# fudan-zvg/S-NeRF

Measured on AMD Instinct MI355X. Metric: rays/sec (train step), higher is better.
Workload: dtype bf16; 1 GPU; S-NeRF path A (MipNerfModel) train step, nuScenes-like 1600x900 rays, 64 proposal + 128 fine evals/ray (192 spp), hidden 1024, rgb_layer 3, cone + contraction + IPE-96

## Files before the change

### snerf_amd/csrc/gemm.hip

```cpp
#include "common.h"
#include <cstdlib>
#include <type_traits>

#define ACT_NONE 0
#define ACT_RELU 1
#define ACT_MASK 2
typedef unsigned short u16x2 __attribute__((ext_vector_type(2)));
#define ACT_RELU_BITS 3
#define ACT_MASK_BITS 4

typedef unsigned u32x4 __attribute__((ext_vector_type(4)));
typedef unsigned u32x2 __attribute__((ext_vector_type(2)));

struct GemmNT {
  const void* A; long lda;
  const void* W; long ldw;
  const float* bias;
  void* Y; long ldy;
  const void* aux; long ldaux;
  float* colsum;
  int M, N, K, n_store, act, out_f32, vec_store;
  float* colsum_ws; int fast_epi;
  int det;
  int dbg;
  int stagger;
  int split;
  int aux_split;
};
__device__ __forceinline__ int split_a_tile(int v) { return 2 * (v / 3) + (v % 3 == 1 ? 1 : 0); }
#ifndef SNERF_PROBE
#define SNERF_PROBE 0
#endif
#define DBG(p, bit) (SNERF_PROBE && ((p).dbg & (bit)))

template <typename T> struct Frag;
template <> struct Frag<float> { typedef f32x4 type; };
template <> struct Frag<__bf16> { typedef bf16x8 type; };

__device__ __forceinline__ void mma32(f32x16& acc, const bf16x8& a, const bf16x8& b) {
  acc = __builtin_amdgcn_mfma_f32_32x32x16_bf16(a, b, acc, 0, 0, 0);
}
__device__ __forceinline__ void mma32(f32x16& acc, const f32x4& a, const f32x4& b) {
#pragma unroll
  for (int s = 0; s < 4; ++s) acc = __builtin_amdgcn_mfma_f32_32x32x2f32(a[s], b[s], acc, 0, 0, 0);
}

typedef _Float16 f16x8 __attribute__((ext_vector_type(8)));
template <bool F16> __device__ __forceinline__ void mma32t(f32x16& acc, const bf16x8& a, const bf16x8& b) {
  if constexpr (F16) acc = __builtin_amdgcn_mfma_f32_32x32x16_f16(__builtin_bit_cast(f16x8, a), __builtin_bit_cast(f16x8, b), acc, 0, 0, 0);
  else acc = __builtin_amdgcn_mfma_f32_32x32x16_bf16(a, b, acc, 0, 0, 0);
}
template <bool F16> __device__ __forceinline__ void mma32t(f32x16& acc, const f32x4& a, const f32x4& b) { mma32(acc, a, b); }
typedef int i32x8 __attribute__((ext_vector_type(8)));
__device__ __forceinline__ void mma8(f32x16& acc, const bf16x8& a0, const bf16x8& a1, const bf16x8& b0, const bf16x8& b1) {
  const i32x8 a = __builtin_bit_cast(i32x8, __builtin_shufflevector(a0, a1, 0, 1, 2, 3, 4, 5, 6, 7, 8, 9, 10, 11, 12, 13, 14, 15));
  const i32x8 b = __builtin_bit_cast(i32x8, __builtin_shufflevector(b0, b1, 0, 1, 2, 3, 4, 5, 6, 7, 8, 9, 10, 11, 12, 13, 14, 15));
  acc = __builtin_amdgcn_mfma_scale_f32_32x32x64_f8f6f4(a, b, acc, 0, 0, 0, 0x74747474, 0, 0x74747474);
}
template <bool F16> __device__ __forceinline__ __bf16 cvt16(float v) {
  if constexpr (F16) return __builtin_bit_cast(__bf16, (_Float16)v);
  else return (__bf16)v;
}
template <bool F16> __device__ __forceinline__ float up16(__bf16 h) {
  if constexpr (F16) return (float)__builtin_bit_cast(_Float16, h);
  else return (float)h;
}
template <bool F16> __device__ __forceinline__ float up16(float x) { return x; }
template <typename T, bool F16> __device__ __forceinline__ T down16(float v) {
  if constexpr (sizeof(T) == 4) return v;
  else return cvt16<F16>(v);
}

typedef __attribute__((address_space(3))) void* lds_ptr_t;
typedef const __attribute__((address_space(1))) void* gbl_ptr_t;

__device__ __forceinline__ void glds16(const void* g, char* lds_wave_base) {
  __builtin_amdgcn_global_load_lds((gbl_ptr_t)g, (lds_ptr_t)lds_wave_base, 16, 0, 0);
}

template <typename T, int BM, int BN, int WM, int WN, bool F16 = false>
__device__ __forceinline__ void nt_epilogue(const GemmNT& p, f32x16 (&acc)[BM / WM / 32][BN / WN / 32], char* smem,
                                            const int m0, const int n0, const int wave, const int lane) {
  typedef typename Frag<T>::type frag_t;
  constexpr int EPC = 16 / (int)sizeof(T);
  constexpr int WTM = BM / WM, WTN = BN / WN, TM = WTM / 32, TN = WTN / 32;
// ... 1150 lines not shown
  variant &= 15;
  hipStream_t s = (hipStream_t)stream;
  const bool p8 = dtype == SNERF_DT_BF16 && (variant & 8) && N % 256 == 0 && K >= 128 && fast && !(colsum != nullptr && act == ACT_RELU) &&
                  (lda * 2 * 256 < (1L << 31)) && (ldw * 2 * 256 < (1L << 31)) && !(split && (act == ACT_MASK || (colsum != nullptr && act == ACT_RELU_BITS))) &&
                  !aux_split &&
                  !(split == 2 && K < 256);
  if (act >= ACT_RELU_BITS && !(p8 && (long)((M + 255) / 256) * 8 * (N / 64) * 256 < (1L << 31)))
    return SNERF_ERR_ARG;
  if (f16) {
    if (p8) return launch_nt8p<true>(p, s);
    if (split == 2) return launch_nt<__bf16, 128, 128, 2, 2, true>(p, s);
    if ((variant & 12) && N % 256 == 0) return launch_nt8<true>(p, s);
    if ((variant & 1) && N % 256 == 0) return launch_nt<__bf16, 256, 256, 2, 4, true>(p, s);
    return launch_nt<__bf16, 128, 128, 2, 2, true>(p, s);
  }
  if (p8) return launch_nt8p(p, s);
  if (dtype == SNERF_DT_BF16 && (variant & 12) && N % 256 == 0) return launch_nt8(p, s);
  if (dtype == SNERF_DT_F32) return launch_nt<float, 128, 128, 2, 2>(p, s);
  if ((variant & 1) && N % 256 == 0) return launch_nt<__bf16, 256, 256, 2, 4>(p, s);
  return launch_nt<__bf16, 128, 128, 2, 2>(p, s);
}

struct GemmTN {
  const void* Z; long ldz;
  const void* X; long ldx;
  float* dW; long ldw;
  const void* zeros;
  int M, N, K, n_valid, k_valid, m_chunk;
  int tiles, slices;
  int split;
  float* part;
  long part_stride;
  int part_ld;
};

template <typename T, bool TR, int TN_STAGES, bool F16 = false>
__global__ __launch_bounds__(256) void gemm_tn_kernel(GemmTN p) {
  extern __shared__ __attribute__((aligned(16))) char smem[];
  constexpr int EPC = 16 / (int)sizeof(T);
  constexpr int ROWB = 128 * (int)sizeof(T);
  constexpr int MT = sizeof(T) == 4 ? 16 : 32;
  constexpr int TILEB = MT * ROWB;
  constexpr int RPI = 1024 / ROWB;
  constexpr int LI = MT / RPI / 4;
  const int tid = threadIdx.x, lane = tid & 63;
  const int wave = __builtin_amdgcn_readfirstlane(tid >> 6);
  const int wn = wave >> 1, wk = wave & 1;
  const int tiles_k = (p.K + 127) / 128;
  const int ntile = p.tiles;
  int slice, tile;
  {
    const int b = (int)blockIdx.x, xcd = b & 7, idx = b >> 3;
    const int full = p.slices >> 3;
    const int extra = p.slices & 7;
    const int mine = full + (xcd < extra ? 1 : 0);
    if (idx >= mine * ntile) return;
    slice = (idx / ntile) * 8 + xcd;
    tile = idx % ntile;
  }
  const int n0 = (tile / tiles_k) * 128, k0 = (tile % tiles_k) * 128;
  const int mbeg = slice * p.m_chunk;
  const int mend = min(p.M, mbeg + p.m_chunk);
  const T* __restrict__ Z = (const T*)p.Z;
  const T* __restrict__ X = (const T*)p.X;
  const int steps = (mend - mbeg + MT - 1) / MT;

// ... 86 lines not shown
        for (int t = 0; t < 2; ++t) {
          const int ca = (wn * 64 + t * 32 + (lane & 31)) * 2, cb = (wk * 64 + t * 32 + (lane & 31)) * 2;
#pragma unroll
          for (int e = 0; e < 8; ++e) {
            a[t].u[e] = *(const unsigned short*)(sZ + (rbase + e) * ROWB + ca);
            b[t].u[e] = *(const unsigned short*)(sX + (rbase + e) * ROWB + cb);
          }
        }
#pragma unroll
        for (int i = 0; i < 2; ++i)
#pragma unroll
          for (int j = 0; j < 2; ++j) mma32t<F16>(acc[i][j], a[i].v, b[j].v);
      }
    }
  }
#pragma unroll
  for (int i = 0; i < 2; ++i)
#pragma unroll
    for (int j = 0; j < 2; ++j) {
      int k = k0 + wk * 64 + j * 32 + (lane & 31);
      if (p.split == 1) k = ((k >> 7) << 6) | (k & 63);
#pragma unroll
      for (int r = 0; r < 16; ++r) {
        int n = n0 + wn * 64 + i * 32 + (r & 3) + 8 * (r >> 2) + 4 * (lane >> 5);
        if (p.split == 1) n = ((n >> 7) << 6) | (n & 63);
        if (n < p.n_valid && k < p.k_valid) {
          if (p.part != nullptr) p.part[(long)slice * p.part_stride + (long)n * p.part_ld + k] = acc[i][j][r];
          else atomicAdd(p.dW + (long)n * p.ldw + k, acc[i][j][r]);
        }
      }
    }
}

template <bool SPLIT, bool F16 = false>
__global__ __launch_bounds__(512) void gemm_tn8_kernel(GemmTN p) {
  extern __shared__ __attribute__((aligned(16))) char smem[];
  typedef __bf16 T;
  typedef __attribute__((address_space(3))) bf16x4* lds_b4;
  constexpr int HALF = 64 * 256;
  const int tid = threadIdx.x, lane = tid & 63;
  const int wave = __builtin_amdgcn_readfirstlane(tid >> 6);
  const int wr = wave >> 2, wc = wave & 3;
  const int tiles_k = (p.K + 255) >> 8, tiles_n = (p.N + 255) >> 8;
  const int ntile = tiles_k * tiles_n;
  const int id = xcd_remap((int)blockIdx.x, (int)gridDim.x);
  const int tile = id % ntile, chunk = id / ntile;
  const int n0 = (tile / tiles_k) << 8, k0 = (tile % tiles_k) << 8;
  const int mbeg = chunk * p.m_chunk;
  const int rows = min(p.M, mbeg + p.m_chunk) - mbeg;
  const int KT = (rows + 63) >> 6;
  const T* __restrict__ Z = (const T*)p.Z + (long)mbeg * p.ldz + n0;
  const bool xhi = !SPLIT && p.split == 2;
  const T* __restrict__ X = (const T*)p.X + (long)mbeg * p.ldx + (xhi ? 2 * k0 : k0);
  const int xcols = xhi ? ((p.K - 1) >> 6) * 128 + ((p.K - 1) & 63) + 1 - 2 * k0 : p.K - k0;
  const int zbytes = (rows - 1) * (int)p.ldz * 2 + (p.N - n0) * 2, xbytes = (rows - 1) * (int)p.ldx * 2 + xcols * 2;
  const int zstep = 64 * (int)p.ldz * 2, xstep = 64 * (int)p.ldx * 2;

  const int lrow = lane >> 4, lch = lane & 15;
  const int lc = (lch ^ (4 * lrow)) * 8;
  constexpr int xhalf = SPLIT ? 128 : 64;
  const int zcol = ((lc >> 6) * 128 + (lc & 63)) * 2;
  const int xcol = SPLIT ? (((lc >> 6) * 128) + ((lc >> 5) & 1) * 32 + (lc & 31)) * 2 : ((lc >> 5) * (xhi ? 128 : 64) + (lc & 31)) * 2;
  int zrel[2], xrel[2];
#pragma unroll
  for (int i = 0; i < 2; ++i) {
    const int r = (wave * 2 + i) * 4 + lrow;
    zrel[i] = r * (int)p.ldz * 2 + zcol;
    xrel[i] = r * (int)p.ldx * 2 + xcol;
  }
  int s_kt = 0;
  auto stage = [&](int db, int which) __attribute__((always_inline)) {
    char* dst = smem + (db * 4 + which) * HALF + wave * 2048;
    if (which < 2) {
      const int off = s_kt * zstep;
      const int left = zbytes - off;
      const __amdgpu_buffer_rsrc_t r = __builtin_amdgcn_make_buffer_rsrc((void*)((const char*)Z + off), 0, left > 0 ? left : 0, 0x00020000);
      __builtin_amdgcn_raw_ptr_buffer_load_lds(r, (lds_ptr_t)dst, 16, zrel[0] + which * 128, 0, 0, 0);
      __builtin_amdgcn_raw_ptr_buffer_load_lds(r, (lds_ptr_t)(dst + 1024), 16, zrel[1] + which * 128, 0, 0, 0);
    } else {
      const int off = s_kt * xstep;
      const int left = xbytes - off;
      const __amdgpu_buffer_rsrc_t r = __builtin_amdgcn_make_buffer_rsrc((void*)((const char*)X + off), 0, left > 0 ? left : 0, 0x00020000);
      __builtin_amdgcn_raw_ptr_buffer_load_lds(r, (lds_ptr_t)dst, 16, xrel[0] + (which - 2) * xhalf, 0, 0, 0);
      __builtin_amdgcn_raw_ptr_buffer_load_lds(r, (lds_ptr_t)(dst + 1024), 16, xrel[1] + (which - 2) * xhalf, 0, 0, 0);
    }
  };

  const int g4 = lane >> 4, pl = lane & 15, prow = pl >> 2;
  const int frow = (8 * (g4 >> 1) + prow) * 256;
  const int fsub = ((pl & 1) << 3);
  int zc[2], xc1;
#pragma unroll
  for (int i2 = 0; i2 < 2; ++i2) zc[i2] = ((((wr * 64 + i2 * 32 + 16 * (g4 & 1)) >> 3) + ((pl & 3) >> 1)) ^ (4 * prow)) << 4;
  xc1 = ((((wc * 32 + 16 * (g4 & 1)) >> 3) + ((pl & 3) >> 1)) ^ (4 * prow)) << 4;
  bf16x8 aF[2][4], bS[2][4];
  const unsigned lds0 = (unsigned)(size_t)smem;
  auto lds_frag = [&](unsigned addr) __attribute__((always_inline)) {
    bf16x4 lo, hi;
    asm volatile("ds_read_b64_tr_b16 %0, %2\n\tds_read_b64_tr_b16 %1, %2 offset:1024" : "=&v"(lo), "=&v"(hi) : "v"(addr));
    return __builtin_shufflevector(lo, hi, 0, 1, 2, 3, 4, 5, 6, 7);
  };
  const unsigned za[2] = {lds0 + frow + zc[0] + fsub, lds0 + frow + zc[1] + fsub};
  const unsigned xa = lds0 + frow + xc1 + fsub;
  auto lds_a = [&](int db, int h, int i2, int ks) __attribute__((always_inline)) {
    return lds_frag(za[i2] + (db * 4 + h) * HALF + ks * 4096);
  };
  auto lds_b = [&](int db, int g, int ks) __attribute__((always_inline)) {
    return lds_frag(xa + (db * 4 + 2 + g) * HALF + ks * 4096);
  };
  f32x16 acc[4][2];
#pragma unroll
  for (int i = 0; i < 4; ++i)
#pragma unroll
    for (int j = 0; j < 2; ++j)
#pragma unroll
      for (int r = 0; r < 16; ++r) acc[i][j][r] = 0.f;

  auto wait_load = [&]() __attribute__((always_inline)) {
    asm volatile("s_waitcnt vmcnt(10)" ::: "memory");
    __builtin_amdgcn_s_waitcnt(0xC07F);
    __builtin_amdgcn_sched_barrier(0);
  };
  auto end_phase = [&]() __attribute__((always_inline)) {
    __builtin_amdgcn_sched_barrier(0);
    __builtin_amdgcn_s_barrier();
    __builtin_amdgcn_sched_barrier(0);
  };

  stage(0, 2); stage(0, 0); stage(0, 3); stage(0, 1);
  ++s_kt;
  stage(1, 3); stage(1, 0); stage(1, 2); stage(1, 1);
  ++s_kt;
  asm volatile("s_waitcnt vmcnt(10)" ::: "memory");
  __builtin_amdgcn_s_barrier();
#pragma unroll
  for (int ks = 0; ks < 4; ++ks) {
    aF[0][ks] = lds_a(0, 0, 0, ks);
    aF[1][ks] = lds_a(0, 0, 1, ks);
    bS[0][ks] = lds_b(0, 0, ks);
  }
  __builtin_amdgcn_s_waitcnt(0xC07F);
  __builtin_amdgcn_sched_barrier(0);
  __builtin_amdgcn_s_barrier();

  auto ktile = [&](auto db_tag) __attribute__((always_inline)) {
    constexpr int db = decltype(db_tag)::value;
    constexpr int F = db, S = 1 - db;
    if (wr == 1) { stage(db, 2 + F); wait_load(); }
#pragma unroll
    for (int ks = 0; ks < 4; ++ks) {
      bS[S][ks] = lds_b(db, S, ks);
      mma32t<F16>(acc[0][F], aF[0][ks], bS[F][ks]);
      mma32t<F16>(acc[1][F], aF[1][ks], bS[F][ks]);
      __builtin_amdgcn_sched_barrier(0);
    }
    if (wr == 0) { stage(db, 2 + F); wait_load(); }
    end_phase();
    if (wr == 1) { stage(db, 0); wait_load(); }
#pragma unroll
    for (int ks = 0; ks < 4; ++ks)
#pragma unroll
      for (int i2 = 0; i2 < 2; ++i2) {
        mma32t<F16>(acc[i2][S], aF[i2][ks], bS[S][ks]);
        aF[i2][ks] = lds_a(db, 1, i2, ks);
        __builtin_amdgcn_sched_barrier(0);
      }
    if (wr == 0) { stage(db, 0); wait_load(); }
    end_phase();
    if (wr == 1) { stage(db, 2 + S); wait_load(); }
    constexpr bool skip3 = S == 1 && SPLIT, skip4 = F == 1 && SPLIT;
#pragma unroll
    for (int ks = 0; ks < 4; ++ks) {
      if constexpr (!skip3) {
        mma32t<F16>(acc[2][S], aF[0][ks], bS[S][ks]);
        mma32t<F16>(acc[3][S], aF[1][ks], bS[S][ks]);
      }
      bS[S][ks] = lds_b(db ^ 1, S, ks);
      __builtin_amdgcn_sched_barrier(0);
    }
    if (wr == 0) { stage(db, 2 + S); wait_load(); }
    end_phase();
    if (wr == 1) { stage(db, 1); ++s_kt; wait_load(); }
#pragma unroll
    for (int ks = 0; ks < 4; ++ks)
#pragma unroll
      for (int i2 = 0; i2 < 2; ++i2) {
        if constexpr (!skip4) mma32t<F16>(acc[2 + i2][F], aF[i2][ks], bS[F][ks]);
        aF[i2][ks] = lds_a(db ^ 1, 0, i2, ks);
        __builtin_amdgcn_sched_barrier(0);
      }
    if (wr == 0) { stage(db, 1); ++s_kt; wait_load(); }
    end_phase();
  };
  for (int t = 0; t < KT; t += 2) {
    ktile(std::integral_constant<int, 0>{});
    if (t + 1 < KT) ktile(std::integral_constant<int, 1>{});
  }
  asm volatile("s_waitcnt vmcnt(0)" ::: "memory");

#pragma unroll
  for (int i = 0; i < 4; ++i)
#pragma unroll
    for (int j = 0; j < 2; ++j) {
      int k = k0 + wc * 64 + j * 32 + (lane & 31);
      if constexpr (SPLIT) {
        if (i >= 2 && j == 1) continue;
        k = k0 + (wc >> 1) * 128 + j * 64 + (wc & 1) * 32 + (lane & 31);
        k = ((k >> 7) << 6) | (k & 63);
      }
#pragma unroll
      for (int r = 0; r < 16; ++r) {
        int n = n0 + wr * 128 + i * 32 + (r & 3) + 8 * (r >> 2) + 4 * (lane >> 5);
        if constexpr (SPLIT) n = ((n >> 7) << 6) | (n & 63);
        if (n < p.n_valid && k < p.k_valid) {
          if (p.part != nullptr) p.part[(long)chunk * p.part_stride + (long)n * p.part_ld + k] = acc[i][j][r];
          else atomicAdd(p.dW + (long)n * p.ldw + k, acc[i][j][r]);
        }
      }
    }
}

template <bool VEC>
__global__ __launch_bounds__(256) void tn_fold_kernel(const float* __restrict__ part, long part_stride, int part_ld, int slices, int n_valid,
                                                      int k_valid, float* __restrict__ dW, long ldw) {
  const int k = (blockIdx.x * 256 + threadIdx.x) * (VEC ? 4 : 1), n = blockIdx.y;
  if (k >= k_valid || n >= n_valid) return;
  const float* src = part + (long)n * part_ld + k;
  if constexpr (VEC) {
    f32x4 s = {0.f, 0.f, 0.f, 0.f};
#pragma unroll 8
    for (int c = 0; c < slices; ++c) s += *(const f32x4*)(src + (long)c * part_stride);
    f32x4* dst = (f32x4*)(dW + (long)n * ldw + k);
    *dst += s;
  } else {
    float s = 0.f;
    for (int c = 0; c < slices; ++c) s += src[(long)c * part_stride];
    dW[(long)n * ldw + k] += s;
  }
}

template <bool VEC>
__global__ __launch_bounds__(1024) void tn_fold_many_kernel(const float* __restrict__ part, long part_stride, int part_ld, int slices, int n_valid,
                                                            int k_valid, float* __restrict__ dW, long ldw) {
  constexpr int G = 16, W = VEC ? 4 : 1;
  __shared__ float sm[G][64][W];
  const int lane = threadIdx.x & 63, g = threadIdx.x >> 6;
  const int kq = k_valid / W;
  const long e = (long)blockIdx.x * 64 + lane;
  const bool live = e < (long)n_valid * kq;
  const int n = live ? (int)(e / kq) : 0, k = live ? (int)(e - (long)n * kq) * W : 0;
  const float* src = part + (long)n * part_ld + k;
  float s[W];
#pragma unroll
  for (int w = 0; w < W; ++w) s[w] = 0.f;
  if (live) {
#pragma unroll 4
    for (int c = g; c < slices; c += G) {
      if constexpr (VEC) { const f32x4 v = *(const f32x4*)(src + (long)c * part_stride); s[0] += v[0]; s[1] += v[1]; s[2] += v[2]; s[3] += v[3]; }
      else s[0] += src[(long)c * part_stride];
    }
  }
#pragma unroll
  for (int w = 0; w < W; ++w) sm[g][lane][w] = s[w];
  __syncthreads();
  if (g == 0 && live) {
    float* dst = dW + (long)n * ldw + k;
#pragma unroll
    for (int w = 0; w < W; ++w) {
      float t = sm[0][lane][w];
#pragma unroll
      for (int q = 1; q < G; ++q) t += sm[q][lane][w];
      dst[w] += t;
    }
  }
}

struct TnPlan {
  bool use8;
  int slices;
  int m_chunk;
  int part_ld;
  long part_stride;
};

static TnPlan tn_plan(int M, int N, int K, long ldz, long ldx, int dtype, int variant, bool fold = false) {
  static int n_cu = 0;
  if (n_cu == 0) {
    int dev = 0;
    hipDeviceProp_t prop;
    n_cu = 256;
    if (hipGetDevice(&dev) == hipSuccess && hipGetDeviceProperties(&prop, dev) == hipSuccess && prop.multiProcessorCount > 0)
      n_cu = prop.multiProcessorCount;
  }
  TnPlan pl{};
  if ((variant & 2) && dtype == SNERF_DT_BF16 && N % 256 == 0 && K >= 256 && M >= 4096 && ldz * 2 * 65 < (1L << 31) && ldx * 2 * 65 < (1L << 31)) {
    const int t8 = (N / 256) * ((K + 255) / 256);
    int ch = n_cu / t8;
    ch = ch < 1 ? 1 : ch;
    long mc = ((long)M + ch - 1) / ch;
    mc = ((mc + 127) / 128) * 128;
    const long lim = (1L << 30) / ((ldz > ldx ? ldz : ldx) * 2);
    if (mc > lim) mc = lim / 128 * 128;
    if (!(fold && M <= 131072 && mc < 512)) {
      pl.use8 = true; pl.m_chunk = (int)mc; pl.slices = (int)((M + mc - 1) / mc);
      pl.part_ld = ((K + 255) / 256) * 256; pl.part_stride = (long)N * pl.part_ld;
      return pl;
    }
  }
  const int tiles = ((N + 127) / 128) * ((K + 127) / 128);
  const int target = (variant & 64) ? 4096 : (variant & 32) ? 2048 : (variant & 16) ? 512 : 1024;
  int chunks = (target + tiles - 1) / tiles;
  int m_chunk = (M + chunks - 1) / chunks;
  m_chunk = ((m_chunk + 255) / 256) * 256;
  const int floor_rows = (fold && M <= 131072) ? 256 : 1024;
  if (m_chunk < floor_rows) m_chunk = floor_rows;
  pl.use8 = false; pl.m_chunk = m_chunk; pl.slices = (M + m_chunk - 1) / m_chunk;
  pl.part_ld = ((K + 127) / 128) * 128; pl.part_stride = (long)(((N + 127) / 128) * 128) * pl.part_ld;
  return pl;
}

static int wgrad_launch(const void* Z, long ldz, const void* X, long ldx, float* dW, long ldw, const void* zeros, int M, int N, int K,
                        int n_valid, int k_valid, int dtype, int variant, float* ws, long ws_floats, void* stream) {
  if (M <= 0) return SNERF_OK;
  const int split = dtype == SNERF_DT_BF16X3;
  if (split) {
    if (N % 128 != 0 || K % 128 != 0 || ws != nullptr) return SNERF_ERR_ARG;
    dtype = SNERF_DT_BF16;
  }
  const int xhi = (variant >> 14) & 1;
  if (xhi && (split || (dtype != SNERF_DT_BF16 && dtype != 2))) return SNERF_ERR_ARG;
  const bool f16 = dtype == 2;
  if (f16) dtype = SNERF_DT_BF16;
  const int epc = dtype == SNERF_DT_F32 ? 4 : 8;
  if (N < epc || K < epc || N % epc || K % epc || ldz % epc || ldx % epc || zeros == nullptr) return SNERF_ERR_ARG;
  const TnPlan pl = tn_plan(M, N, K, ldz, ldx, dtype, variant, ws != nullptr);
  if (ws != nullptr && ws_floats < pl.part_stride * pl.slices) return SNERF_ERR_ARG;
  GemmTN p{Z, ldz, X, ldx, dW, ldw, zeros, M, N, K, n_valid, k_valid, pl.m_chunk, 0, pl.slices, split ? 1 : (xhi ? 2 : 0), ws, pl.part_stride, pl.part_ld};
  if (pl.use8) {
    static bool attr_set = false;
    if (!attr_set) {
      hipFuncSetAttribute((const void*)gemm_tn8_kernel<false>, hipFuncAttributeMaxDynamicSharedMemorySize, 8 * 64 * 256);
      hipFuncSetAttribute((const void*)gemm_tn8_kernel<true>, hipFuncAttributeMaxDynamicSharedMemorySize, 8 * 64 * 256);
      attr_set = true;
    }
    const int t8 = (N / 256) * ((K + 255) / 256);
    if (f16) {
      static bool attr16 = false;
      if (!attr16) { hipFuncSetAttribute((const void*)gemm_tn8_kernel<false, true>, hipFuncAttributeMaxDynamicSharedMemorySize, 8 * 64 * 256); attr16 = true; }
      hipLaunchKernelGGL((gemm_tn8_kernel<false, true>), dim3(t8 * pl.slices), dim3(512), 8 * 64 * 256, (hipStream_t)stream, p);
    } else if (split) hipLaunchKernelGGL(gemm_tn8_kernel<true>, dim3(t8 * pl.slices), dim3(512), 8 * 64 * 256, (hipStream_t)stream, p);
    else hipLaunchKernelGGL(gemm_tn8_kernel<false>, dim3(t8 * pl.slices), dim3(512), 8 * 64 * 256, (hipStream_t)stream, p);
  } else {
    const int tiles = ((N + 127) / 128) * ((K + 127) / 128);
    p.tiles = tiles;
    const bool deep = (variant & 128) != 0;
    const int lds = (deep ? 4 : 2) * 2 * 8192;
    static bool tn_attr_set = false;
    if (!tn_attr_set) {
      hipFuncSetAttribute((const void*)gemm_tn_kernel<float, false, 4>, hipFuncAttributeMaxDynamicSharedMemorySize, 4 * 2 * 8192);
      hipFuncSetAttribute((const void*)gemm_tn_kernel<__bf16, true, 4>, hipFuncAttributeMaxDynamicSharedMemorySize, 4 * 2 * 8192);
      hipFuncSetAttribute((const void*)gemm_tn_kernel<__bf16, false, 4>, hipFuncAttributeMaxDynamicSharedMemorySize, 4 * 2 * 8192);
      tn_attr_set = true;
    }
    dim3 grid(8 * ((pl.slices + 7) / 8) * tiles);
    const bool tr = (variant & 1) && dtype == SNERF_DT_BF16 && (N % 128 == 0) && (K % 128 == 0);
    hipStream_t st = (hipStream_t)stream;
    if (f16) {
      static bool tn16_attr = false;
      if (!tn16_attr) {
        hipFuncSetAttribute((const void*)gemm_tn_kernel<__bf16, true, 4, true>, hipFuncAttributeMaxDynamicSharedMemorySize, 4 * 2 * 8192);
        hipFuncSetAttribute((const void*)gemm_tn_kernel<__bf16, false, 4, true>, hipFuncAttributeMaxDynamicSharedMemorySize, 4 * 2 * 8192);
        tn16_attr = true;
      }
      if (tr) { if (deep) hipLaunchKernelGGL((gemm_tn_kernel<__bf16, true, 4, true>), grid, dim3(256), lds, st, p);
                else hipLaunchKernelGGL((gemm_tn_kernel<__bf16, true, 2, true>), grid, dim3(256), lds, st, p); }
      else { if (deep) hipLaunchKernelGGL((gemm_tn_kernel<__bf16, false, 4, true>), grid, dim3(256), lds, st, p);
             else hipLaunchKernelGGL((gemm_tn_kernel<__bf16, false, 2, true>), grid, dim3(256), lds, st, p); }
    } else if (dtype == SNERF_DT_F32) {
      if (deep) hipLaunchKernelGGL((gemm_tn_kernel<float, false, 4>), grid, dim3(256), lds, st, p);
      else hipLaunchKernelGGL((gemm_tn_kernel<float, false, 2>), grid, dim3(256), lds, st, p);
    } else if (dtype == SNERF_DT_BF16 && tr) {
      if (deep) hipLaunchKernelGGL((gemm_tn_kernel<__bf16, true, 4>), grid, dim3(256), lds, st, p);
      else hipLaunchKernelGGL((gemm_tn_kernel<__bf16, true, 2>), grid, dim3(256), lds, st, p);
    } else if (dtype == SNERF_DT_BF16) {
      if (deep) hipLaunchKernelGGL((gemm_tn_kernel<__bf16, false, 4>), grid, dim3(256), lds, st, p);
      else hipLaunchKernelGGL((gemm_tn_kernel<__bf16, false, 2>), grid, dim3(256), lds, st, p);
    } else return SNERF_ERR_ARG;
  }
  if (ws != nullptr) {
    const bool vec = k_valid % 4 == 0 && pl.part_ld % 4 == 0 && pl.part_stride % 4 == 0 && ldw % 4 == 0 && ((size_t)dW & 15) == 0 && ((size_t)ws & 15) == 0;
    if (pl.slices > 32) {
      const long pieces = (long)n_valid * (vec ? k_valid / 4 : k_valid);
      const dim3 fg((unsigned)((pieces + 63) / 64));
      if (vec) hipLaunchKernelGGL(tn_fold_many_kernel<true>, fg, dim3(1024), 0, (hipStream_t)stream, ws, pl.part_stride, pl.part_ld, pl.slices, n_valid, k_valid, dW, ldw);
      else hipLaunchKernelGGL(tn_fold_many_kernel<false>, fg, dim3(1024), 0, (hipStream_t)stream, ws, pl.part_stride, pl.part_ld, pl.slices, n_valid, k_valid, dW, ldw);
    } else if (vec)
      hipLaunchKernelGGL(tn_fold_kernel<true>, dim3((k_valid / 4 + 255) / 256, n_valid), dim3(256), 0, (hipStream_t)stream, ws, pl.part_stride,
                         pl.part_ld, pl.slices, n_valid, k_valid, dW, ldw);
    else
      hipLaunchKernelGGL(tn_fold_kernel<false>, dim3((k_valid + 255) / 256, n_valid), dim3(256), 0, (hipStream_t)stream, ws, pl.part_stride,
                         pl.part_ld, pl.slices, n_valid, k_valid, dW, ldw);
  }
  return snerf_check_launch();
}

extern "C" int snerf_linear_wgrad(const void* Z, long ldz, const void* X, long ldx, float* dW, long ldw, const void* zeros,
                                  int M, int N, int K, int n_valid, int k_valid, int dtype, int variant, void* stream) {
  return wgrad_launch(Z, ldz, X, ldx, dW, ldw, zeros, M, N, K, n_valid, k_valid, dtype, variant, nullptr, 0, stream);
}

extern "C" long snerf_linear_wgrad_ws_floats(int M, int N, int K, long ldz, long ldx, int dtype, int variant) {
  if (M <= 0 || N <= 0 || K <= 0) return 0;
  if (dtype == 2) dtype = SNERF_DT_BF16;
  const TnPlan pl = tn_plan(M, N, K, ldz, ldx, dtype, variant, true);
  return pl.part_stride * pl.slices;
}

extern "C" int snerf_linear_wgrad_det(const void* Z, long ldz, const void* X, long ldx, float* dW, long ldw, const void* zeros, int M, int N,
                                      int K, int n_valid, int k_valid, int dtype, int variant, float* ws, long ws_floats, void* stream) {
  if (ws == nullptr) return SNERF_ERR_ARG;
  return wgrad_launch(Z, ldz, X, ldx, dW, ldw, zeros, M, N, K, n_valid, k_valid, dtype, variant, ws, ws_floats, stream);
}
```

Before: 162,800 rays/s.

## Schedule ragged-K edge tiles separately in bf16 weight-gradient GEMM

When K is not a multiple of 256 (remainder at most 128), the tn8 weight-gradient kernel now gives the partial last K tile its own blocks. These use a dedicated edge path that loads half-width X columns and skips MFMAs for dead wave columns. A planner picks separate M-chunk counts for full and edge tiles so the grid better fills the CUs, and the fold kernels sum a different slice count for the edge columns. The goal is to stop wasting half of each edge tile's MMA work and to balance load, at the cost of more planner complexity and a possibly larger workspace.

```diff
diff --git a/snerf_amd/csrc/gemm.hip b/snerf_amd/csrc/gemm.hip
--- a/snerf_amd/csrc/gemm.hip
+++ b/snerf_amd/csrc/gemm.hip
@@ -1,4 +1,5 @@
 #include "common.h"
+#include <climits>
 #include <cstdlib>
 #include <type_traits>
 
@@ -1267,6 +1268,7 @@
   float* part;
   long part_stride;
   int part_ld;
+  int edge_first, m_chunk_edge;
 };
 
 template <typename T, bool TR, int TN_STAGES, bool F16 = false>
@@ -1419,22 +1421,16 @@
     }
 }
 
-template <bool SPLIT, bool F16 = false>
-__global__ __launch_bounds__(512) void gemm_tn8_kernel(GemmTN p) {
-  extern __shared__ __attribute__((aligned(16))) char smem[];
+template <bool SPLIT, bool F16, bool EDGE>
+__device__ __forceinline__ void gemm_tn8_tile(const GemmTN& p, char* smem, const int n0, const int k0, const int chunk, const int m_chunk) {
   typedef __bf16 T;
   typedef __attribute__((address_space(3))) bf16x4* lds_b4;
   constexpr int HALF = 64 * 256;
   const int tid = threadIdx.x, lane = tid & 63;
   const int wave = __builtin_amdgcn_readfirstlane(tid >> 6);
   const int wr = wave >> 2, wc = wave & 3;
-  const int tiles_k = (p.K + 255) >> 8, tiles_n = (p.N + 255) >> 8;
-  const int ntile = tiles_k * tiles_n;
-  const int id = xcd_remap((int)blockIdx.x, (int)gridDim.x);
-  const int tile = id % ntile, chunk = id / ntile;
-  const int n0 = (tile / tiles_k) << 8, k0 = (tile % tiles_k) << 8;
-  const int mbeg = chunk * p.m_chunk;
-  const int rows = min(p.M, mbeg + p.m_chunk) - mbeg;
+  const int mbeg = chunk * m_chunk;
+  const int rows = min(p.M, mbeg + m_chunk) - mbeg;
   const int KT = (rows + 63) >> 6;
   const T* __restrict__ Z = (const T*)p.Z + (long)mbeg * p.ldz + n0;
   const bool xhi = !SPLIT && p.split == 2;
@@ -1445,9 +1441,18 @@
 
   const int lrow = lane >> 4, lch = lane & 15;
   const int lc = (lch ^ (4 * lrow)) * 8;
-  constexpr int xhalf = SPLIT ? 128 : 64;
+  constexpr int xhalf = EDGE ? 0 : SPLIT ? 128 : 64;
   const int zcol = ((lc >> 6) * 128 + (lc & 63)) * 2;
-  const int xcol = SPLIT ? (((lc >> 6) * 128) + ((lc >> 5) & 1) * 32 + (lc & 31)) * 2 : ((lc >> 5) * (xhi ? 128 : 64) + (lc & 31)) * 2;
+  const int xcol = EDGE ? lc * 2 : SPLIT ? (((lc >> 6) * 128) + ((lc >> 5) & 1) * 32 + (lc & 31)) * 2 : ((lc >> 5) * (xhi ? 128 : 64) + (lc & 31)) * 2;
+  int xedge[2] = {0, 0};
+  bool live[2] = {true, true};
+  if constexpr (EDGE) {
+#pragma unroll
+    for (int g = 0; g < 2; ++g) {
+      xedge[g] = k0 + g * 128 + lc < p.K ? g * 256 : 0x60000000;
+      live[g] = k0 + g * 128 + wc * 32 < p.K;
+    }
+  }
   int zrel[2], xrel[2];
 #pragma unroll
   for (int i = 0; i < 2; ++i) {
@@ -1468,8 +1473,9 @@
       const int off = s_kt * xstep;
       const int left = xbytes - off;
       const __amdgpu_buffer_rsrc_t r = __builtin_amdgcn_make_buffer_rsrc((void*)((const char*)X + off), 0, left > 0 ? left : 0, 0x00020000);
-      __builtin_amdgcn_raw_ptr_buffer_load_lds(r, (lds_ptr_t)dst, 16, xrel[0] + (which - 2) * xhalf, 0, 0, 0);
-      __builtin_amdgcn_raw_ptr_buffer_load_lds(r, (lds_ptr_t)(dst + 1024), 16, xrel[1] + (which - 2) * xhalf, 0, 0, 0);
+      const int xo = EDGE ? xedge[which - 2] : (which - 2) * xhalf;
+      __builtin_amdgcn_raw_ptr_buffer_load_lds(r, (lds_ptr_t)dst, 16, xrel[0] + xo, 0, 0, 0);
+      __builtin_amdgcn_raw_ptr_buffer_load_lds(r, (lds_ptr_t)(dst + 1024), 16, xrel[1] + xo, 0, 0, 0);
     }
   };
 
@@ -1537,8 +1543,10 @@
 #pragma unroll
     for (int ks = 0; ks < 4; ++ks) {
       bS[S][ks] = lds_b(db, S, ks);
-      mma32t<F16>(acc[0][F], aF[0][ks], bS[F][ks]);
-      mma32t<F16>(acc[1][F], aF[1][ks], bS[F][ks]);
+      if (!EDGE || live[F]) {
+        mma32t<F16>(acc[0][F], aF[0][ks], bS[F][ks]);
+        mma32t<F16>(acc[1][F], aF[1][ks], bS[F][ks]);
+      }
       __builtin_amdgcn_sched_barrier(0);
     }
     if (wr == 0) { stage(db, 2 + F); wait_load(); }
@@ -1548,7 +1556,7 @@
     for (int ks = 0; ks < 4; ++ks)
 #pragma unroll
       for (int i2 = 0; i2 < 2; ++i2) {
-        mma32t<F16>(acc[i2][S], aF[i2][ks], bS[S][ks]);
+        if (!EDGE || live[S]) mma32t<F16>(acc[i2][S], aF[i2][ks], bS[S][ks]);
         aF[i2][ks] = lds_a(db, 1, i2, ks);
         __builtin_amdgcn_sched_barrier(0);
       }
@@ -1558,7 +1566,7 @@
     constexpr bool skip3 = S == 1 && SPLIT, skip4 = F == 1 && SPLIT;
 #pragma unroll
     for (int ks = 0; ks < 4; ++ks) {
-      if constexpr (!skip3) {
+      if (!skip3 && (!EDGE || live[S])) {
         mma32t<F16>(acc[2][S], aF[0][ks], bS[S][ks]);
         mma32t<F16>(acc[3][S], aF[1][ks], bS[S][ks]);
       }
@@ -1572,7 +1580,7 @@
     for (int ks = 0; ks < 4; ++ks)
 #pragma unroll
       for (int i2 = 0; i2 < 2; ++i2) {
-        if constexpr (!skip4) mma32t<F16>(acc[2 + i2][F], aF[i2][ks], bS[F][ks]);
+        if (!skip4 && (!EDGE || live[F])) mma32t<F16>(acc[2 + i2][F], aF[i2][ks], bS[F][ks]);
         aF[i2][ks] = lds_a(db ^ 1, 0, i2, ks);
         __builtin_amdgcn_sched_barrier(0);
       }
@@ -1589,7 +1597,8 @@
   for (int i = 0; i < 4; ++i)
 #pragma unroll
     for (int j = 0; j < 2; ++j) {
-      int k = k0 + wc * 64 + j * 32 + (lane & 31);
+      int k = EDGE ? k0 + j * 128 + wc * 32 + (lane & 31) : k0 + wc * 64 + j * 32 + (lane & 31);
+      if (EDGE && !live[j]) continue;
       if constexpr (SPLIT) {
         if (i >= 2 && j == 1) continue;
         k = k0 + (wc >> 1) * 128 + j * 64 + (wc & 1) * 32 + (lane & 31);
@@ -1607,11 +1616,35 @@
     }
 }
 
+template <bool SPLIT, bool F16 = false>
+__global__ __launch_bounds__(512) void gemm_tn8_kernel(GemmTN p) {
+  extern __shared__ __attribute__((aligned(16))) char smem[];
+  const int tiles_n = (p.N + 255) >> 8;
+  int tiles_k = (p.K + 255) >> 8;
+  int id = xcd_remap((int)blockIdx.x, (int)gridDim.x);
+  if constexpr (!SPLIT) {
+    if (p.edge_first > 0) {
+      const int G = (int)gridDim.x, E = G - p.edge_first;
+      const int e = (int)((long)id * E / G);
+      if ((int)((long)(id + 1) * E / G) > e) {
+        gemm_tn8_tile<false, F16, true>(p, smem, (e % tiles_n) << 8, (tiles_k - 1) << 8, e / tiles_n, p.m_chunk_edge);
+        return;
+      }
+      id -= e;
+      --tiles_k;
+    }
+  }
+  const int ntile = tiles_k * tiles_n;
+  const int tile = id % ntile, chunk = id / ntile;
+  gemm_tn8_tile<SPLIT, F16, false>(p, smem, (tile / tiles_k) << 8, (tile % tiles_k) << 8, chunk, p.m_chunk);
+}
+
 template <bool VEC>
 __global__ __launch_bounds__(256) void tn_fold_kernel(const float* __restrict__ part, long part_stride, int part_ld, int slices, int n_valid,
-                                                      int k_valid, float* __restrict__ dW, long ldw) {
+                                                      int k_valid, float* __restrict__ dW, long ldw, int k_split, int slices_edge) {
   const int k = (blockIdx.x * 256 + threadIdx.x) * (VEC ? 4 : 1), n = blockIdx.y;
   if (k >= k_valid || n >= n_valid) return;
+  if (k >= k_split) slices = slices_edge;
   const float* src = part + (long)n * part_ld + k;
   if constexpr (VEC) {
     f32x4 s = {0.f, 0.f, 0.f, 0.f};
@@ -1628,7 +1661,7 @@
 
 template <bool VEC>
 __global__ __launch_bounds__(1024) void tn_fold_many_kernel(const float* __restrict__ part, long part_stride, int part_ld, int slices, int n_valid,
-                                                            int k_valid, float* __restrict__ dW, long ldw) {
+                                                            int k_valid, float* __restrict__ dW, long ldw, int k_split, int slices_edge) {
   constexpr int G = 16, W = VEC ? 4 : 1;
   __shared__ float sm[G][64][W];
   const int lane = threadIdx.x & 63, g = threadIdx.x >> 6;
@@ -1637,6 +1670,7 @@
   const bool live = e < (long)n_valid * kq;
   const int n = live ? (int)(e / kq) : 0, k = live ? (int)(e - (long)n * kq) * W : 0;
   const float* src = part + (long)n * part_ld + k;
+  if (k >= k_split) slices = slices_edge;
   float s[W];
 #pragma unroll
   for (int w = 0; w < W; ++w) s[w] = 0.f;
@@ -1668,9 +1702,39 @@
   int m_chunk;
   int part_ld;
   long part_stride;
+  int slices_edge;
+  int m_chunk_edge;
+  int ws_slices() const { return slices > slices_edge ? slices : slices_edge; }
 };
 
-static TnPlan tn_plan(int M, int N, int K, long ldz, long ldx, int dtype, int variant, bool fold = false) {
+constexpr double TN8_EDGE_COST = 0.57;
+static void tn_plan_ragged(TnPlan& pl, int M, int N, int K, long ldz, long ldx, int n_cu, bool fold, int probe) {
+  const int kr = K % 256;
+  if (kr == 0 || kr > 128 || probe == 15) return;
+  const int n_e = N / 256, n_f = n_e * (K / 256);
+  if (n_f + n_e > n_cu) return;
+  int s_e = 0, s_f = 0;
+  double best = 0.;
+  for (int e = 1; n_f + n_e * e <= n_cu; ++e) {
+    if (probe != 0 && e != probe) continue;
+    const int f = (n_cu - n_e * e) / n_f;
+    const double t = 1. / f > TN8_EDGE_COST / e ? 1. / f : TN8_EDGE_COST / e;
+    if (s_e == 0 || t < best) { best = t; s_e = e; s_f = f; }
+  }
+  if (s_e == 0) return;
+  const long lim = (1L << 30) / ((ldz > ldx ? ldz : ldx) * 2) / 128 * 128;
+  long mc[2] = {((long)M + s_f - 1) / s_f, ((long)M + s_e - 1) / s_e};
+  for (long& m : mc) {
+    m = ((m + 127) / 128) * 128;
+    if (m > lim) m = lim;
+  }
+  if (fold && M <= 131072 && mc[0] < 512) return;
+  pl.m_chunk = (int)mc[0]; pl.slices = (int)((M + mc[0] - 1) / mc[0]);
+  pl.m_chunk_edge = (int)mc[1]; pl.slices_edge = (int)((M + mc[1] - 1) / mc[1]);
+}
+
+
+static TnPlan tn_plan(int M, int N, int K, long ldz, long ldx, int dtype, int variant, bool fold = false, bool plain_bf16 = false) {
   static int n_cu = 0;
   if (n_cu == 0) {
     int dev = 0;
@@ -1691,6 +1755,7 @@
     if (!(fold && M <= 131072 && mc < 512)) {
       pl.use8 = true; pl.m_chunk = (int)mc; pl.slices = (int)((M + mc - 1) / mc);
       pl.part_ld = ((K + 255) / 256) * 256; pl.part_stride = (long)N * pl.part_ld;
+      if (plain_bf16) tn_plan_ragged(pl, M, N, K, ldz, ldx, n_cu, fold, (variant >> 20) & 15);
       return pl;
     }
   }
@@ -1720,9 +1785,11 @@
   if (f16) dtype = SNERF_DT_BF16;
   const int epc = dtype == SNERF_DT_F32 ? 4 : 8;
   if (N < epc || K < epc || N % epc || K % epc || ldz % epc || ldx % epc || zeros == nullptr) return SNERF_ERR_ARG;
-  const TnPlan pl = tn_plan(M, N, K, ldz, ldx, dtype, variant, ws != nullptr);
-  if (ws != nullptr && ws_floats < pl.part_stride * pl.slices) return SNERF_ERR_ARG;
-  GemmTN p{Z, ldz, X, ldx, dW, ldw, zeros, M, N, K, n_valid, k_valid, pl.m_chunk, 0, pl.slices, split ? 1 : (xhi ? 2 : 0), ws, pl.part_stride, pl.part_ld};
+  const TnPlan pl = tn_plan(M, N, K, ldz, ldx, dtype, variant, ws != nullptr, !split && !xhi && !f16);
+  if (ws != nullptr && ws_floats < pl.part_stride * pl.ws_slices()) return SNERF_ERR_ARG;
+  const int k_split = pl.slices_edge > 0 ? K / 256 * 256 : INT_MAX;
+  GemmTN p{Z, ldz, X, ldx, dW, ldw, zeros, M, N, K, n_valid, k_valid, pl.m_chunk, 0, pl.slices, split ? 1 : (xhi ? 2 : 0), ws, pl.part_stride, pl.part_ld,
+           pl.slices_edge > 0 ? (N / 256) * (K / 256) * pl.slices : 0, pl.m_chunk_edge};
   if (pl.use8) {
     static bool attr_set = false;
     if (!attr_set) {
@@ -1730,13 +1797,13 @@
       hipFuncSetAttribute((const void*)gemm_tn8_kernel<true>, hipFuncAttributeMaxDynamicSharedMemorySize, 8 * 64 * 256);
       attr_set = true;
     }
-    const int t8 = (N / 256) * ((K + 255) / 256);
+    const int grid8 = pl.slices_edge > 0 ? p.edge_first + (N / 256) * pl.slices_edge : (N / 256) * ((K + 255) / 256) * pl.slices;
     if (f16) {
       static bool attr16 = false;
       if (!attr16) { hipFuncSetAttribute((const void*)gemm_tn8_kernel<false, true>, hipFuncAttributeMaxDynamicSharedMemorySize, 8 * 64 * 256); attr16 = true; }
-      hipLaunchKernelGGL((gemm_tn8_kernel<false, true>), dim3(t8 * pl.slices), dim3(512), 8 * 64 * 256, (hipStream_t)stream, p);
-    } else if (split) hipLaunchKernelGGL(gemm_tn8_kernel<true>, dim3(t8 * pl.slices), dim3(512), 8 * 64 * 256, (hipStream_t)stream, p);
-    else hipLaunchKernelGGL(gemm_tn8_kernel<false>, dim3(t8 * pl.slices), dim3(512), 8 * 64 * 256, (hipStream_t)stream, p);
+      hipLaunchKernelGGL((gemm_tn8_kernel<false, true>), dim3(grid8), dim3(512), 8 * 64 * 256, (hipStream_t)stream, p);
+    } else if (split) hipLaunchKernelGGL(gemm_tn8_kernel<true>, dim3(grid8), dim3(512), 8 * 64 * 256, (hipStream_t)stream, p);
+    else hipLaunchKernelGGL(gemm_tn8_kernel<false>, dim3(grid8), dim3(512), 8 * 64 * 256, (hipStream_t)stream, p);
   } else {
     const int tiles = ((N + 127) / 128) * ((K + 127) / 128);
     p.tiles = tiles;
@@ -1779,14 +1846,14 @@
     if (pl.slices > 32) {
       const long pieces = (long)n_valid * (vec ? k_valid / 4 : k_valid);
       const dim3 fg((unsigned)((pieces + 63) / 64));
-      if (vec) hipLaunchKernelGGL(tn_fold_many_kernel<true>, fg, dim3(1024), 0, (hipStream_t)stream, ws, pl.part_stride, pl.part_ld, pl.slices, n_valid, k_valid, dW, ldw);
-      else hipLaunchKernelGGL(tn_fold_many_kernel<false>, fg, dim3(1024), 0, (hipStream_t)stream, ws, pl.part_stride, pl.part_ld, pl.slices, n_valid, k_valid, dW, ldw);
+      if (vec) hipLaunchKernelGGL(tn_fold_many_kernel<true>, fg, dim3(1024), 0, (hipStream_t)stream, ws, pl.part_stride, pl.part_ld, pl.slices, n_valid, k_valid, dW, ldw, k_split, pl.slices_edge);
+      else hipLaunchKernelGGL(tn_fold_many_kernel<false>, fg, dim3(1024), 0, (hipStream_t)stream, ws, pl.part_stride, pl.part_ld, pl.slices, n_valid, k_valid, dW, ldw, k_split, pl.slices_edge);
     } else if (vec)
       hipLaunchKernelGGL(tn_fold_kernel<true>, dim3((k_valid / 4 + 255) / 256, n_valid), dim3(256), 0, (hipStream_t)stream, ws, pl.part_stride,
-                         pl.part_ld, pl.slices, n_valid, k_valid, dW, ldw);
+                         pl.part_ld, pl.slices, n_valid, k_valid, dW, ldw, k_split, pl.slices_edge);
     else
       hipLaunchKernelGGL(tn_fold_kernel<false>, dim3((k_valid + 255) / 256, n_valid), dim3(256), 0, (hipStream_t)stream, ws, pl.part_stride,
-                         pl.part_ld, pl.slices, n_valid, k_valid, dW, ldw);
+                         pl.part_ld, pl.slices, n_valid, k_valid, dW, ldw, k_split, pl.slices_edge);
   }
   return snerf_check_launch();
 }
@@ -1798,9 +1865,10 @@
 
 extern "C" long snerf_linear_wgrad_ws_floats(int M, int N, int K, long ldz, long ldx, int dtype, int variant) {
   if (M <= 0 || N <= 0 || K <= 0) return 0;
+  const bool plain = dtype == SNERF_DT_BF16 && !((variant >> 14) & 1);
   if (dtype == 2) dtype = SNERF_DT_BF16;
-  const TnPlan pl = tn_plan(M, N, K, ldz, ldx, dtype, variant, true);
-  return pl.part_stride * pl.slices;
+  const TnPlan pl = tn_plan(M, N, K, ldz, ldx, dtype, variant, true, plain);
+  return pl.part_stride * pl.ws_slices();
 }
 
 extern "C" int snerf_linear_wgrad_det(const void* Z, long ldz, const void* X, long ldx, float* dW, long ldw, const void* zeros, int M, int N,
```

New measurement: 161,100 rays/s, median of 2. -1.0%, worse.

## Switch weight-gradient GEMM to 16x16x32 MFMA with remapped LDS staging layout

Applied to the files above, without the earlier changes.

Rewrites the TN weight-gradient kernel's inner loops to use 16x16x32 bf16/f16 MFMA tiles instead of 32x32x16, with the accumulator split into 8x4 f32x4 fragments. It remaps which rows each lane stages into LDS and uses compile-time offsets in the transposed LDS reads, so address arithmetic folds into instruction immediates. The epilogue is rewritten to match the new fragment layout. The aim is better LDS-read and MFMA interleaving and fewer VALU address ops. The cost is more MFMA instructions per tile and a different bank-conflict profile.

```diff
diff --git a/snerf_amd/csrc/gemm.hip b/snerf_amd/csrc/gemm.hip
--- a/snerf_amd/csrc/gemm.hip
+++ b/snerf_amd/csrc/gemm.hip
@@ -1,6 +1,7 @@
 #include "common.h"
 #include <cstdlib>
 #include <type_traits>
+#include <utility>
 
 #define ACT_NONE 0
 #define ACT_RELU 1
@@ -51,6 +52,19 @@
   else acc = __builtin_amdgcn_mfma_f32_32x32x16_bf16(a, b, acc, 0, 0, 0);
 }
 template <bool F16> __device__ __forceinline__ void mma32t(f32x16& acc, const f32x4& a, const f32x4& b) { mma32(acc, a, b); }
+template <bool F16> __device__ __forceinline__ void mma16t(f32x4& acc, const bf16x8& a, const bf16x8& b) {
+  if constexpr (F16) acc = __builtin_amdgcn_mfma_f32_16x16x32_f16(__builtin_bit_cast(f16x8, a), __builtin_bit_cast(f16x8, b), acc, 0, 0, 0);
+  else acc = __builtin_amdgcn_mfma_f32_16x16x32_bf16(a, b, acc, 0, 0, 0);
+}
+template <int V> using ic_ = std::integral_constant<int, V>;
+template <int... I, class Fn> __device__ __forceinline__ void sfor_seq(std::integer_sequence<int, I...>, Fn&& f) { (f(std::integral_constant<int, I>{}), ...); }
+template <int N, class Fn> __device__ __forceinline__ void sfor(Fn&& f) { sfor_seq(std::make_integer_sequence<int, N>{}, f); }
+template <int OFF, int SECOND> __device__ __forceinline__ bf16x8 lds_tr_frag(unsigned addr) {
+  static_assert(OFF >= 0 && OFF + SECOND < 65536 && OFF % 8 == 0 && SECOND % 8 == 0, "ds offset field");
+  bf16x4 lo, hi;
+  asm volatile("ds_read_b64_tr_b16 %0, %2 offset:%3\n\tds_read_b64_tr_b16 %1, %2 offset:%4" : "=&v"(lo), "=&v"(hi) : "v"(addr), "n"(OFF), "n"(OFF + SECOND));
+  return __builtin_shufflevector(lo, hi, 0, 1, 2, 3, 4, 5, 6, 7);
+}
 typedef int i32x8 __attribute__((ext_vector_type(8)));
 __device__ __forceinline__ void mma8(f32x16& acc, const bf16x8& a0, const bf16x8& a1, const bf16x8& b0, const bf16x8& b1) {
   const i32x8 a = __builtin_bit_cast(i32x8, __builtin_shufflevector(a0, a1, 0, 1, 2, 3, 4, 5, 6, 7, 8, 9, 10, 11, 12, 13, 14, 15));
@@ -1443,17 +1457,17 @@
   const int zbytes = (rows - 1) * (int)p.ldz * 2 + (p.N - n0) * 2, xbytes = (rows - 1) * (int)p.ldx * 2 + xcols * 2;
   const int zstep = 64 * (int)p.ldz * 2, xstep = 64 * (int)p.ldx * 2;
 
-  const int lrow = lane >> 4, lch = lane & 15;
-  const int lc = (lch ^ (4 * lrow)) * 8;
+  const int srow = 32 * (wave >> 2) + 16 * (wave & 1) + 4 * ((wave >> 1) & 1) + 8 * ((lane >> 3) & 1) + ((lane >> 1) & 3);
+  const int lc0 = 16 * (lane >> 4) + 8 * (lane & 1);
   constexpr int xhalf = SPLIT ? 128 : 64;
-  const int zcol = ((lc >> 6) * 128 + (lc & 63)) * 2;
-  const int xcol = SPLIT ? (((lc >> 6) * 128) + ((lc >> 5) & 1) * 32 + (lc & 31)) * 2 : ((lc >> 5) * (xhi ? 128 : 64) + (lc & 31)) * 2;
   int zrel[2], xrel[2];
 #pragma unroll
   for (int i = 0; i < 2; ++i) {
-    const int r = (wave * 2 + i) * 4 + lrow;
-    zrel[i] = r * (int)p.ldz * 2 + zcol;
-    xrel[i] = r * (int)p.ldx * 2 + xcol;
+    const int lc = lc0 + 64 * i;
+    const int zcol = ((lc >> 6) * 128 + (lc & 63)) * 2;
+    const int xcol = SPLIT ? (((lc >> 6) * 128) + ((lc >> 5) & 1) * 32 + (lc & 31)) * 2 : ((lc >> 5) * (xhi ? 128 : 64) + (lc & 31)) * 2;
+    zrel[i] = srow * (int)p.ldz * 2 + zcol;
+    xrel[i] = srow * (int)p.ldx * 2 + xcol;
   }
   int s_kt = 0;
   auto stage = [&](int db, int which) __attribute__((always_inline)) {
@@ -1473,35 +1487,20 @@
     }
   };
 
-  const int g4 = lane >> 4, pl = lane & 15, prow = pl >> 2;
-  const int frow = (8 * (g4 >> 1) + prow) * 256;
-  const int fsub = ((pl & 1) << 3);
-  int zc[2], xc1;
-#pragma unroll
-  for (int i2 = 0; i2 < 2; ++i2) zc[i2] = ((((wr * 64 + i2 * 32 + 16 * (g4 & 1)) >> 3) + ((pl & 3) >> 1)) ^ (4 * prow)) << 4;
-  xc1 = ((((wc * 32 + 16 * (g4 & 1)) >> 3) + ((pl & 3) >> 1)) ^ (4 * prow)) << 4;
-  bf16x8 aF[2][4], bS[2][4];
-  const unsigned lds0 = (unsigned)(size_t)smem;
-  auto lds_frag = [&](unsigned addr) __attribute__((always_inline)) {
-    bf16x4 lo, hi;
-    asm volatile("ds_read_b64_tr_b16 %0, %2\n\tds_read_b64_tr_b16 %1, %2 offset:1024" : "=&v"(lo), "=&v"(hi) : "v"(addr));
-    return __builtin_shufflevector(lo, hi, 0, 1, 2, 3, 4, 5, 6, 7);
-  };
-  const unsigned za[2] = {lds0 + frow + zc[0] + fsub, lds0 + frow + zc[1] + fsub};
-  const unsigned xa = lds0 + frow + xc1 + fsub;
-  auto lds_a = [&](int db, int h, int i2, int ks) __attribute__((always_inline)) {
-    return lds_frag(za[i2] + (db * 4 + h) * HALF + ks * 4096);
-  };
-  auto lds_b = [&](int db, int g, int ks) __attribute__((always_inline)) {
-    return lds_frag(xa + (db * 4 + 2 + g) * HALF + ks * 4096);
-  };
-  f32x16 acc[4][2];
-#pragma unroll
-  for (int i = 0; i < 4; ++i)
-#pragma unroll
-    for (int j = 0; j < 2; ++j)
-#pragma unroll
-      for (int r = 0; r < 16; ++r) acc[i][j][r] = 0.f;
+  bf16x8 aF[4][2], bS[2][2][2];
+  const unsigned lds0 = (unsigned)(size_t)smem + 2048 * (lane >> 5) + 8 * (lane & 31);
+  const unsigned za = lds0 + wr * 1024, xa = lds0 + wc * 512;
+  auto lds_a = [&](auto db, auto h, auto nb, auto s) __attribute__((always_inline)) {
+    return lds_tr_frag<decltype(h)::value * HALF + decltype(s)::value * 8192 + decltype(nb)::value * 256, 4096>(za + decltype(db)::value * 4 * HALF);
+  };
+  auto lds_b = [&](auto db, auto g, auto kb, auto s) __attribute__((always_inline)) {
+    return lds_tr_frag<(2 + decltype(g)::value) * HALF + decltype(s)::value * 8192 + decltype(kb)::value * 256, 4096>(xa + decltype(db)::value * 4 * HALF);
+  };
+  f32x4 acc[8][4];
+#pragma unroll
+  for (int i = 0; i < 8; ++i)
+#pragma unroll
+    for (int j = 0; j < 4; ++j) acc[i][j] = f32x4{0.f, 0.f, 0.f, 0.f};
 
   auto wait_load = [&]() __attribute__((always_inline)) {
     asm volatile("s_waitcnt vmcnt(10)" ::: "memory");
@@ -1520,12 +1519,14 @@
   ++s_kt;
   asm volatile("s_waitcnt vmcnt(10)" ::: "memory");
   __builtin_amdgcn_s_barrier();
-#pragma unroll
-  for (int ks = 0; ks < 4; ++ks) {
-    aF[0][ks] = lds_a(0, 0, 0, ks);
-    aF[1][ks] = lds_a(0, 0, 1, ks);
-    bS[0][ks] = lds_b(0, 0, ks);
-  }
+  sfor<8>([&](auto t) __attribute__((always_inline)) {
+    constexpr int s = decltype(t)::value >> 2, nb = decltype(t)::value & 3;
+    aF[nb][s] = lds_a(ic_<0>{}, ic_<0>{}, ic_<nb>{}, ic_<s>{});
+  });
+  sfor<4>([&](auto t) __attribute__((always_inline)) {
+    constexpr int s = decltype(t)::value >> 1, kb = decltype(t)::value & 1;
+    bS[0][kb][s] = lds_b(ic_<0>{}, ic_<0>{}, ic_<kb>{}, ic_<s>{});
+  });
   __builtin_amdgcn_s_waitcnt(0xC07F);
   __builtin_amdgcn_sched_barrier(0);
   __builtin_amdgcn_s_barrier();
@@ -1534,48 +1535,44 @@
     constexpr int db = decltype(db_tag)::value;
     constexpr int F = db, S = 1 - db;
     if (wr == 1) { stage(db, 2 + F); wait_load(); }
-#pragma unroll
-    for (int ks = 0; ks < 4; ++ks) {
-      bS[S][ks] = lds_b(db, S, ks);
-      mma32t<F16>(acc[0][F], aF[0][ks], bS[F][ks]);
-      mma32t<F16>(acc[1][F], aF[1][ks], bS[F][ks]);
+    sfor<4>([&](auto t) __attribute__((always_inline)) {
+      constexpr int s = decltype(t)::value >> 1, kb = decltype(t)::value & 1;
+      bS[S][kb][s] = lds_b(ic_<db>{}, ic_<S>{}, ic_<kb>{}, ic_<s>{});
+      sfor<4>([&](auto nb) __attribute__((always_inline)) { mma16t<F16>(acc[nb][2 * F + kb], aF[nb][s], bS[F][kb][s]); });
       __builtin_amdgcn_sched_barrier(0);
-    }
+    });
     if (wr == 0) { stage(db, 2 + F); wait_load(); }
     end_phase();
     if (wr == 1) { stage(db, 0); wait_load(); }
-#pragma unroll
-    for (int ks = 0; ks < 4; ++ks)
-#pragma unroll
-      for (int i2 = 0; i2 < 2; ++i2) {
-        mma32t<F16>(acc[i2][S], aF[i2][ks], bS[S][ks]);
-        aF[i2][ks] = lds_a(db, 1, i2, ks);
-        __builtin_amdgcn_sched_barrier(0);
-      }
+    sfor<8>([&](auto t) __attribute__((always_inline)) {
+      constexpr int s = decltype(t)::value >> 2, nb = decltype(t)::value & 3;
+      mma16t<F16>(acc[nb][2 * S], aF[nb][s], bS[S][0][s]);
+      mma16t<F16>(acc[nb][2 * S + 1], aF[nb][s], bS[S][1][s]);
+      aF[nb][s] = lds_a(ic_<db>{}, ic_<1>{}, ic_<nb>{}, ic_<s>{});
+      __builtin_amdgcn_sched_barrier(0);
+    });
     if (wr == 0) { stage(db, 0); wait_load(); }
     end_phase();
     if (wr == 1) { stage(db, 2 + S); wait_load(); }
     constexpr bool skip3 = S == 1 && SPLIT, skip4 = F == 1 && SPLIT;
-#pragma unroll
-    for (int ks = 0; ks < 4; ++ks) {
-      if constexpr (!skip3) {
-        mma32t<F16>(acc[2][S], aF[0][ks], bS[S][ks]);
-        mma32t<F16>(acc[3][S], aF[1][ks], bS[S][ks]);
-      }
-      bS[S][ks] = lds_b(db ^ 1, S, ks);
+    sfor<4>([&](auto t) __attribute__((always_inline)) {
+      constexpr int s = decltype(t)::value >> 1, kb = decltype(t)::value & 1;
+      if constexpr (!skip3) sfor<4>([&](auto nb) __attribute__((always_inline)) { mma16t<F16>(acc[4 + nb][2 * S + kb], aF[nb][s], bS[S][kb][s]); });
+      bS[S][kb][s] = lds_b(ic_<db ^ 1>{}, ic_<S>{}, ic_<kb>{}, ic_<s>{});
       __builtin_amdgcn_sched_barrier(0);
-    }
+    });
     if (wr == 0) { stage(db, 2 + S); wait_load(); }
     end_phase();
     if (wr == 1) { stage(db, 1); ++s_kt; wait_load(); }
-#pragma unroll
-    for (int ks = 0; ks < 4; ++ks)
-#pragma unroll
-      for (int i2 = 0; i2 < 2; ++i2) {
-        if constexpr (!skip4) mma32t<F16>(acc[2 + i2][F], aF[i2][ks], bS[F][ks]);
-        aF[i2][ks] = lds_a(db ^ 1, 0, i2, ks);
-        __builtin_amdgcn_sched_barrier(0);
-      }
+    sfor<8>([&](auto t) __attribute__((always_inline)) {
+      constexpr int s = decltype(t)::value >> 2, nb = decltype(t)::value & 3;
+      if constexpr (!skip4) {
+        mma16t<F16>(acc[4 + nb][2 * F], aF[nb][s], bS[F][0][s]);
+        mma16t<F16>(acc[4 + nb][2 * F + 1], aF[nb][s], bS[F][1][s]);
+      }
+      aF[nb][s] = lds_a(ic_<db ^ 1>{}, ic_<0>{}, ic_<nb>{}, ic_<s>{});
+      __builtin_amdgcn_sched_barrier(0);
+    });
     if (wr == 0) { stage(db, 1); ++s_kt; wait_load(); }
     end_phase();
   };
@@ -1585,26 +1582,27 @@
   }
   asm volatile("s_waitcnt vmcnt(0)" ::: "memory");
 
-#pragma unroll
-  for (int i = 0; i < 4; ++i)
-#pragma unroll
-    for (int j = 0; j < 2; ++j) {
-      int k = k0 + wc * 64 + j * 32 + (lane & 31);
+  sfor<32>([&](auto t) __attribute__((always_inline)) {
+    constexpr int i = decltype(t)::value >> 2, j = decltype(t)::value & 3;
+    if constexpr (!(SPLIT && i >= 4 && j >= 2)) {
+      int k = k0 + wc * 64 + j * 16 + (lane & 15);
       if constexpr (SPLIT) {
-        if (i >= 2 && j == 1) continue;
-        k = k0 + (wc >> 1) * 128 + j * 64 + (wc & 1) * 32 + (lane & 31);
+        k = k0 + (wc >> 1) * 128 + (j >> 1) * 64 + (wc & 1) * 32 + (j & 1) * 16 + (lane & 15);
         k = ((k >> 7) << 6) | (k & 63);
       }
-#pragma unroll
-      for (int r = 0; r < 16; ++r) {
-        int n = n0 + wr * 128 + i * 32 + (r & 3) + 8 * (r >> 2) + 4 * (lane >> 5);
+      const f32x4 v = acc[i][j];
+      const float vr[4] = {v[0], v[1], v[2], v[3]};
+#pragma unroll
+      for (int r = 0; r < 4; ++r) {
+        int n = n0 + wr * 128 + i * 16 + 4 * (lane >> 4) + r;
         if constexpr (SPLIT) n = ((n >> 7) << 6) | (n & 63);
         if (n < p.n_valid && k < p.k_valid) {
-          if (p.part != nullptr) p.part[(long)chunk * p.part_stride + (long)n * p.part_ld + k] = acc[i][j][r];
-          else atomicAdd(p.dW + (long)n * p.ldw + k, acc[i][j][r]);
-        }
-      }
-    }
+          if (p.part != nullptr) p.part[(long)chunk * p.part_stride + (long)n * p.part_ld + k] = vr[r];
+          else atomicAdd(p.dW + (long)n * p.ldw + k, vr[r]);
+        }
+      }
+    }
+  });
 }
 
 template <bool VEC>
```

After: 159,000 rays/s before, 158,900 rays/s after. About the same (-0.1%).
